# princeton-computational-imaging/Neural-Volume-Super-Resolution

Measured on AMD Instinct MI355X. Metric: rendered rays/sec (64+128 samples) at 800x800 Lego-like view, higher is better.
Workload: dtype f32 as 2 f16 limbs (3 MFMA products, f32 acc); 1 GPU; Blender-'lego'-like 800x800 view, 64 coarse + 128 fine samples, tri-plane decoder (3x800^2x48 + 32^2x48 planes, 4+4x128 MLP), 1 view per GPU per step; partition=view

## Files before the change

include/nvsr.h:

```cpp
#ifndef NVSR_H
#define NVSR_H
#include <stdint.h>

#ifdef __cplusplus
extern "C" {
#endif

typedef void* nvsr_stream_t;

typedef enum {
    NVSR_OK = 0,
    NVSR_ERR_SHAPE = 1,
    NVSR_ERR_LAUNCH = 2,
    NVSR_ERR_NULL = 3,
    NVSR_ERR_ALIGN = 4
} nvsr_status;

#define NVSR_PLANE_CHANNELS 48
#define NVSR_DEC_CHANNELS 128
#define NVSR_DEC_LAYERS 4
#define NVSR_DECODER_NATURAL_FLOATS 130564
#define NVSR_DECODER_PACKED_F32_FLOATS 130576
#define NVSR_DECODER_PACKED_FLOATS 453136
#define NVSR_DECODER_PACKED_BWD_FLOATS 487424
// ... 10 lines not shown

#define NVSR_ARITH_INHERIT (-1)
#define NVSR_ARITH_INVALID (-2)
#define NVSR_ARITH_F32 0
#define NVSR_ARITH_F16 1
#define NVSR_ARITH_F16X2 2
#define NVSR_ARITH_BF16X3 3
#define NVSR_ARITH_DEFAULT NVSR_ARITH_F16X2
int nvsr_get_decoder_arithmetic(void);
int nvsr_set_decoder_arithmetic(int mode);
int nvsr_set_range_flag(uint32_t* device_word);
uint32_t* nvsr_get_range_flag(void);
int nvsr_release_render_scratch(void);
int64_t nvsr_render_scratch_bytes(void);
int nvsr_internal_group_order(const int* trips, int64_t G, int S, int* out, nvsr_stream_t stream);
int nvsr_internal_copy_group_order(int* dst, int64_t G, nvsr_stream_t stream);
int nvsr_internal_live_order(int* live_n, int64_t N, int S, nvsr_stream_t stream);
int nvsr_internal_colour_order_bins(void);
int nvsr_internal_copy_live_counts(int* dst, int64_t N, nvsr_stream_t stream);
int nvsr_internal_point_order(const int* entries, const float* lists, const float* rays, int64_t N, int S, int bands, int* points, int* steps, int* offsets,
                              nvsr_stream_t stream);
int nvsr_internal_point_bands(void);
int nvsr_internal_copy_point_steps(int* dst, int64_t G, nvsr_stream_t stream);
int64_t nvsr_occupancy_words(int G);
int64_t nvsr_occupancy_workspace_floats(int G, int K);
int nvsr_occupancy_build(const nvsr_scene* scene, const float* packed_decoder, int G, int K, float threshold, int dilate, int arithmetic, uint32_t* grid,
                         float* workspace, nvsr_stream_t stream);
int nvsr_render_pass_occupancy_arith(const nvsr_scene* scene, const float* packed_decoder, int64_t N, int S, const float* rays, const float* z, int lindisp,
                                     int white_bkgd, float* rgb, float* disp, float* acc, float* weights, float* depth, const uint32_t* grid, int G, int arithmetic,
                                     nvsr_stream_t stream);
int nvsr_render_rays_occupancy_arith(const nvsr_scene* scene, const float* packed_coarse, const float* packed_fine, int64_t N, int Nc, int Nf,
                                     const float* rays, int lindisp, int white_bkgd, const float* t_rand, const float* u, float* rgb_c, float* disp_c,
                                     float* acc_c, float* rgb_f, float* disp_f, float* acc_f, float* workspace, const uint32_t* grid_coarse, int G_coarse,
                                     const uint32_t* grid_fine, int G_fine, int arithmetic, nvsr_stream_t stream);
int nvsr_internal_occupancy_probes(const nvsr_scene* scene, int G, int K, float* x, nvsr_stream_t stream);
int nvsr_internal_occupancy_cull(const nvsr_scene* scene, int64_t N, int S, const float* rays, const float* z, int lindisp, const uint32_t* grid, int G, int* kept,
                                 int* kept_n, nvsr_stream_t stream);
int nvsr_internal_copy_kept_counts(int* dst, int64_t N, nvsr_stream_t stream);
int nvsr_limb_gemm_probe(int arithmetic, int K, const float* W, const float* X, float* Y, nvsr_stream_t stream);
#define NVSR_CONV_ARITH_DEFAULT NVSR_ARITH_F16X2
int nvsr_get_conv_arithmetic(void);
int nvsr_set_conv_arithmetic(int mode);

int nvsr_plane_to_channel_last(const float* nchw, float* nhwc, int C, int H, int W, nvsr_stream_t stream);
int nvsr_plane_from_channel_last(const float* nhwc, float* nchw, int C, int H, int W, nvsr_stream_t stream);

// ... 349 lines not shown
```

neural-volume-super-resolution_amd/build.py:

```python
import glob
import os
import shutil
import subprocess

PKG_DIR = os.path.dirname(os.path.abspath(__file__))
CSRC = os.path.join(PKG_DIR, "csrc")
LIB_PATH = os.path.join(PKG_DIR, "libnvsr_hip.so")
HIPCC_FLAGS = ["--offload-arch=gfx950", "-O3", "-std=c++17", "-fPIC", "-shared", "-ffp-contract=off"]


def sources():
    return sorted(glob.glob(os.path.join(CSRC, "*.hip")))


STAMP_PATH = LIB_PATH + ".flags"


def _flag_stamp():
    extra = os.environ.get("NVSR_EXTRA_HIPCC_FLAGS", "").split()
    return " ".join(HIPCC_FLAGS) + " | " + " ".join("%s:%s" % kv for kv in sorted((k, ",".join(v)) for k, v in PER_FILE_FLAGS.items())) + " | " + " ".join(extra)


def _stamp_matches():
    try:
        with open(STAMP_PATH) as f:
            return f.read() == _flag_stamp()
    except OSError:
        return False


def _stale():
    if not os.path.exists(LIB_PATH) or not _stamp_matches():
        return True
    t = os.path.getmtime(LIB_PATH)
    deps = sources() + glob.glob(os.path.join(CSRC, "*.h")) + glob.glob(os.path.join(PKG_DIR, "..", "include", "*.h")) + [os.path.abspath(__file__)]
    return any(os.path.getmtime(p) > t for p in deps)


_PAIR_FLAGS = ["-fno-slp-vectorize", "-mllvm", "-pragma-unroll-threshold=1000000"]
_SR_FLAGS = ["-mllvm", "-enable-post-misched=0"]
PER_FILE_FLAGS = {"render3.hip": _PAIR_FLAGS, "decode_pair.hip": _PAIR_FLAGS, "decode_limb.hip": ["-fno-slp-vectorize"], "render_bwd_limb.hip": ["-fno-slp-vectorize"],
                  "sr.hip": _SR_FLAGS, "sr_bwd.hip": _SR_FLAGS}
OBJ_DIR = os.path.join(CSRC, "_obj")


def _compile_one(hipcc, src, verbose):
    obj = os.path.join(OBJ_DIR, os.path.basename(src) + ".o")
    deps = [src] + glob.glob(os.path.join(CSRC, "*.h")) + glob.glob(os.path.join(PKG_DIR, "..", "include", "*.h")) + [os.path.abspath(__file__)]
    stamp = obj + ".flags"
    same_flags = os.path.exists(stamp) and open(stamp).read() == _flag_stamp()
    if same_flags and os.path.exists(obj) and all(os.path.getmtime(d) <= os.path.getmtime(obj) for d in deps):
        return obj
    flags = [f for f in HIPCC_FLAGS if f != "-shared"] + PER_FILE_FLAGS.get(os.path.basename(src), [])
    flags += os.environ.get("NVSR_EXTRA_HIPCC_FLAGS", "").split()
    cmd = [hipcc] + flags + ["-c", src, "-o", obj]
    if verbose:
        print(" ".join(cmd))
    subprocess.check_call(cmd)
    with open(obj + ".flags", "w") as f:
        f.write(_flag_stamp())
    return obj


def build_extension(force=False, verbose=False, out_path=None):
# ... 54 lines not shown
```

neural-volume-super-resolution_amd/capi.py:

```python
import ctypes as C
import os

import torch

from .build import LIB_PATH as _DEFAULT_LIB_PATH

LIB_PATH = os.environ.get("NVSR_HIP_LIB", _DEFAULT_LIB_PATH)

PLANE_CHANNELS = 48
DEC_CHANNELS = 128
DECODER_NATURAL_FLOATS = 130564
DECODER_PACKED_FLOATS = 453136
DECODER_PACKED_BWD_FLOATS = 487424
MIP_NERF_NATURAL_FLOATS = 81092
MIP_NERF_RECORD_FLOATS = 767
MIP_NERF_GRAD_RECORD_FLOATS = 708
PE_NERF_NATURAL_FLOATS = 81476
PE_NERF_RECORD_FLOATS = 770
PE_NERF_GRAD_RECORD_FLOATS = 708
MSE_PAIR_MAX_ELEMS = 1 << 22

_STATUS = {1: "NVSR_ERR_SHAPE (argument out of the supported range)", 2: "NVSR_ERR_LAUNCH (kernel launch failed)",
           3: "NVSR_ERR_NULL (required pointer is NULL)", 4: "NVSR_ERR_ALIGN (pointer not 16-byte aligned)"}

# ... 158 lines not shown
    "nvsr_ray_points": ([_i64, _i, _vp, _vp, _vp, _vp], _i),
    "nvsr_render_shared_workspace_floats": ([_i64, _i, _i], _i64),
    "nvsr_render_rays_shared_arith": ([C.POINTER(Scene), _vp, _i64, _i, _i, _vp, _i, _i, _vp, _vp, _vp, _vp, _vp, _vp, _vp, _vp, _vp, _vp, _vp, _i, _vp], _i),
    "nvsr_shared_merge": ([_i64, _i, _i, _vp, _i, _vp, _vp, _vp, _vp, _vp, _vp], _i),
    "nvsr_release_render_scratch": ([], _i),
    "nvsr_render_scratch_bytes": ([], _i64),
    "nvsr_internal_group_order": ([_vp, _i64, _i, _vp, _vp], _i),
    "nvsr_internal_copy_group_order": ([_vp, _i64, _vp], _i),
    "nvsr_internal_live_order": ([_vp, _i64, _i, _vp], _i),
    "nvsr_internal_colour_order_bins": ([], _i),
    "nvsr_internal_copy_live_counts": ([_vp, _i64, _vp], _i),
    "nvsr_internal_point_bands": ([], _i),
    "nvsr_internal_copy_point_steps": ([_vp, _i64, _vp], _i),
    "nvsr_internal_point_order": ([_vp, _vp, _vp, _i64, _i, _i, _vp, _vp, _vp, _vp], _i),
    "nvsr_occupancy_words": ([_i], _i64),
    "nvsr_occupancy_workspace_floats": ([_i, _i], _i64),
    "nvsr_occupancy_build": ([C.POINTER(Scene), _vp, _i, _i, C.c_float, _i, _i, _vp, _vp, _vp], _i),
    "nvsr_render_pass_occupancy_arith": ([C.POINTER(Scene), _vp, _i64, _i, _vp, _vp, _i, _i, _vp, _vp, _vp, _vp, _vp, _vp, _i, _i, _vp], _i),
    "nvsr_render_rays_occupancy_arith": ([C.POINTER(Scene), _vp, _vp, _i64, _i, _i, _vp, _i, _i, _vp, _vp, _vp, _vp, _vp, _vp, _vp, _vp, _vp, _vp, _i, _vp, _i,
                                          _i, _vp], _i),
    "nvsr_internal_occupancy_probes": ([C.POINTER(Scene), _i, _i, _vp, _vp], _i),
    "nvsr_internal_occupancy_cull": ([C.POINTER(Scene), _i64, _i, _vp, _vp, _i, _vp, _i, _vp, _vp, _vp], _i),
    "nvsr_internal_copy_kept_counts": ([_vp, _i64, _vp], _i),
    "nvsr_set_sr_plane_interp": ([_i], _i),
    "nvsr_get_sr_plane_interp": ([], _i),
    "nvsr_set_sr_align_corners": ([_i], _i),
    "nvsr_get_sr_align_corners": ([], _i),
    "nvsr_render_pass_arith": ([C.POINTER(Scene), _vp, _i64, _i, _vp, _vp, _vp, _i, _vp, _vp, _vp, _vp, _vp, _vp, _i, _vp], _i),
    "nvsr_decode_rays_arith": ([C.POINTER(Scene), _vp, _i64, _i, _vp, _vp, _vp, _vp, _vp, _i, _vp], _i),
    "nvsr_render_rays_arith": ([C.POINTER(Scene), _vp, _vp, _i64, _i, _i, _vp, _i, _i, _vp, _vp, _vp, _vp, _vp, _vp, _vp, _vp, _vp,
                                _vp, _vp, _i, _vp], _i),
    "nvsr_render_pass_backward_gates_arith": ([C.POINTER(Scene), _vp, _vp, _i64, _i, _vp, _vp, _vp, _vp, C.POINTER(C.c_void_p), _vp, _vp, _i, _vp], _i),
    "nvsr_decoder_weight_grad_arith": ([_i64, _i, _vp, _vp, _i, _vp], _i),
    "nvsr_conv3x3_arith": ([_vp, _i, _i, _i, _vp, _i, _i, _vp, _vp, _i, _i, _vp], _i),
    "nvsr_conv3x3_dgrad_arith": ([_vp, _i, _i, _i, _vp, _i, _vp, _i, _i, _vp], _i),
    "nvsr_conv3x3_wgrad_arith": ([_vp, _vp, _i, _i, _i, _i, C.c_float, _vp, _vp, _i, _vp], _i),
    "nvsr_edsr_forward_batch_arith": ([_vp, _i, _i, _i, _i, _vp, _i, _i, _i, _i, _vp, _vp, _i, _vp], _i),
    "nvsr_edsr_forward_train_arith": ([_vp, _i, _i, _i, _vp, _i, _i, _i, _i, _vp, _vp, _i, _vp], _i),
    "nvsr_edsr_backward_arith": ([_vp, _i, _i, _i, _vp, _vp, _i, _i, _i, _i, _vp, _vp, _vp, _vp, _i, _vp], _i),
    "nvsr_planes_sr_arith": ([_vp, _i, _i, _i, _vp, _i, _i, _i, _i, _i, _fp, _vp, _vp, _vp, _vp, _i, _vp], _i),
    "nvsr_planes_sr_batch_arith": ([C.POINTER(C.c_void_p), _i, _i, _i, _i, _vp, _i, _i, _i, _i, _i, _fp, _vp, _vp, C.POINTER(C.c_void_p), _vp, _i, _vp], _i),
    "nvsr_planes_sr_train_arith": ([_vp, _i, _i, _i, _vp, _i, _i, _i, _i, _i, _fp, _vp, _vp, _vp, _vp, _vp, _i, _vp], _i),
    "nvsr_planes_sr_backward_arith": ([_i, _i, _i, _vp, _vp, _i, _i, _i, _i, _i, _fp, _vp, _vp, _vp, _vp, _vp, _i, _vp], _i),
    "nvsr_planes_sr_batch_ex": ([C.POINTER(C.c_void_p), _i, _i, _i, _i, _vp, _i, _i, _i, _i, _i, _fp, _vp, _vp, C.POINTER(C.c_void_p), _vp, _i, _i, _i, _vp], _i),
    "nvsr_planes_sr_batch_keep_floats": ([_i, _i, _i, _i, _i, _i, _i, _i, _fp], _i64),
    "nvsr_planes_sr_batch_workspace_floats": ([_i, _i, _i, _i, _i, _i, _i, _i, _fp], _i64),
# ... 248 lines not shown
```

neural-volume-super-resolution_amd/csrc/colour_order.h:

```cpp
#pragma once
#include "tile_pair.h"

namespace nvsr {

constexpr int ORDER_SHIFT = 12, ORDER_RAYS = 1 << ORDER_SHIFT, ORDER_BINS = 32;
constexpr int ORDER_MAX_S = 1 << (31 - ORDER_SHIFT);
static_assert(ORDER_RAYS % RAYS2 == 0, "a block of the ray order is a whole number of workgroups");

#ifndef NVSR_POINT_BANDS
#define NVSR_POINT_BANDS 0
#endif
constexpr int POINT_BANDS = NVSR_POINT_BANDS, POINT_NONE = -1, POINT_VIEW_FLOATS = 2 * HALF_C;
static_assert(RAYS2 <= 256 && ORDER_MAX_S <= (1 << 24), "a slot and a list index share an entry");

struct LiveLists { float* z; float* w; int* n; int* slot; int* trip; int* pts; int* steps; float* views; };

struct KeptLists { int* idx; int* n; int* slot; int* trip; };

enum class PassRoute { Fused, TwoPhase, Occupancy };
PassRoute acquire_pass_scratch(int64_t N, int S, hipStream_t stream, bool raw_out, bool want_kept, bool launch, LiveLists& live, KeptLists& kept);
void launch_colour_order(const LiveLists& ll, int64_t N, int S, hipStream_t stream);
void launch_kept_order(const KeptLists& kl, int64_t N, int S, hipStream_t stream);
void launch_point_order(const LiveLists& ll, const float* rays_nf, int64_t N, int S, hipStream_t stream);

}
```

neural-volume-super-resolution_amd/csrc/colour_order.hip:

```cpp
#include "colour_order.h"
#include "occupancy.h"
#include "nvsr_internal.h"

#include <cstdlib>
#include <mutex>
#include <vector>

namespace nvsr {

constexpr int SORT_TPB = 1024, SORT_WAVES = SORT_TPB / 64, SORT_ROUNDS = 4, SORT_MAX = SORT_TPB * SORT_ROUNDS;
template <int NKEYS>
__device__ __forceinline__ void counting_sort(const int (&key)[SORT_ROUNDS], int nkeys, int n, int (&start)[SORT_ROUNDS], int (&place)[SORT_ROUNDS],
                                              int (&len)[SORT_ROUNDS]) {
    static_assert(NKEYS <= SORT_TPB, "one thread per key sums the tables");
    __shared__ int cnt_s[NKEYS * SORT_WAVES];
    __shared__ int tot_s[NKEYS], start_s[NKEYS];
    const int wave = threadIdx.x >> 6, lane = threadIdx.x & 63;
    const unsigned long long below = (1ull << lane) - 1ull;
    for (int b = 0; b <= nkeys; ++b) {
        int c = 0;
#pragma unroll
        for (int r = 0; r < SORT_ROUNDS; ++r) c += __popcll(__ballot(key[r] == b));
        if (lane == 0) cnt_s[b * SORT_WAVES + wave] = c;
    }
// ... 145 lines not shown
    if (base + j < nsteps * RAYS2) out[base + j] = POINT_NONE;
    if (j == 0) { steps[blockIdx.x] = nsteps; offs[blockIdx.x] = (int)blockIdx.x * S; }
    __syncthreads();
    for (int t = 0; t < nsteps; ++t) {
        const int e = out[t * RAYS2 + j];
        const bool valid = e != POINT_NONE;
        const int sl = (int)((unsigned)e >> 24), kk = e & 0xffffff;
        kmin_s[j] = 0x7fffffff; cnt_s[j] = 0;
        __syncthreads();
        if (valid) { atomicMin(&kmin_s[sl], kk); atomicAdd(&cnt_s[sl], 1); }
        __syncthreads();
        int total;
        start_s[j] = scan(cnt_s[j], 0, total);
        __syncthreads();
        stage_s[valid ? start_s[sl] + (kk - kmin_s[sl]) : j] = e;
        __syncthreads();
        out[t * RAYS2 + j] = stage_s[j];
    }
}

namespace {
enum { LISTS, GROUP, POINTS, VIEWS, KEPT, KEPT_GROUP, N_BUFFERS };
struct Buffer { void* p; size_t bytes; };
struct Launch { int64_t N; int* n; int* steps; int64_t kept_N; int* kept; };
struct Scratch { int device; hipStream_t stream; Buffer buf[N_BUFFERS]; Launch last; };
std::mutex g_live_mutex;
std::vector<Scratch> g_live;

Scratch* find_scratch(int device, hipStream_t stream) {
    for (Scratch& c : g_live)
        if (c.device == device && c.stream == stream) return &c;
    return nullptr;
}

bool grow(Scratch& e, int which, size_t bytes) {
    Buffer& b = e.buf[which];
    if (b.bytes >= bytes) return true;
    if (b.p) (void)hipFree(b.p);
    b = Buffer{};
    e.last = Launch{};
    void* p = nullptr;
    if (hipMalloc(&p, bytes) != hipSuccess) { (void)hipGetLastError(); return false; }
    b = Buffer{p, bytes};
    return true;
}

int64_t groups_of(int64_t N) { return (N + RAYS2 - 1) / RAYS2; }
// ... 55 lines not shown
    live.w = live.z + rows;
    live.n = reinterpret_cast<int*>(live.w + rows);
    live.slot = static_cast<int*>(e->buf[GROUP].p);
    live.trip = live.slot + G;
    const size_t npts = G * RAYS2 * (size_t)S;
    if (!env_starts("NVSR_COLOUR_POINTS", '0') && G * (size_t)S <= 0x7fffffffu && grow(*e, POINTS, (npts + 2 * G) * sizeof(int)) &&
        grow(*e, VIEWS, G * RAYS2 * POINT_VIEW_FLOATS * sizeof(float))) {
        live.pts = static_cast<int*>(e->buf[POINTS].p);
        live.steps = live.pts + npts;
        live.views = static_cast<float*>(e->buf[VIEWS].p);
    }
    PassRoute route = PassRoute::TwoPhase;
    if (want_kept && grow(*e, KEPT_GROUP, 2 * G * sizeof(int)) && grow(*e, KEPT, (rows + (size_t)N) * sizeof(int))) {
        kept.idx = static_cast<int*>(e->buf[KEPT].p);
        kept.n = kept.idx + rows;
        kept.slot = static_cast<int*>(e->buf[KEPT_GROUP].p);
        kept.trip = kept.slot + G;
        route = PassRoute::Occupancy;
    }
    if (launch) e->last = route == PassRoute::Occupancy ? Launch{N, live.n, live.steps, N, kept.n} : Launch{N, live.n, live.steps, e->last.kept_N, e->last.kept};
    return route;
}

static void launch_orders(int* n, int* trip, int* slot, int64_t N, int S, hipStream_t stream) {
    launch_live_order(n, N, S, env_starts("NVSR_COLOUR_ORDER", '0') ? 0 : ORDER_BINS, trip, stream);
    launch_group_order(trip, groups_of(N), S, slot, stream);
}
void launch_kept_order(const KeptLists& kl, int64_t N, int S, hipStream_t stream) { launch_orders(kl.n, kl.trip, kl.slot, N, S, stream); }
void launch_colour_order(const LiveLists& ll, int64_t N, int S, hipStream_t stream) { launch_orders(ll.n, ll.trip, ll.slot, N, S, stream); }

void launch_point_order(const LiveLists& ll, const float* rays_nf, int64_t N, int S, hipStream_t stream) {
    launch_point_order(ll.n, ll.z, rays_nf, N, S, POINT_BANDS, ll.pts, ll.steps, ll.steps + groups_of(N), stream);
}

}

using namespace nvsr;

extern "C" int nvsr_internal_colour_order_bins(void) { return ORDER_BINS; }
extern "C" int nvsr_internal_live_order(int* live_n, int64_t N, int S, nvsr_stream_t stream) {
    if (!live_n) return NVSR_ERR_NULL;
    if (N < 1 || S < 1 || S >= ORDER_MAX_S || (N + ORDER_RAYS - 1) / ORDER_RAYS > 0x7fffffff) return NVSR_ERR_SHAPE;
    launch_live_order(live_n, N, S, ORDER_BINS, nullptr, (hipStream_t)stream);
    return NVSR_CHECK_LAUNCH();
}
extern "C" int nvsr_internal_copy_live_counts(int* dst, int64_t N, nvsr_stream_t stream) {
    return copy_left_behind(dst, N, stream, [N](const Scratch& c) { return c.last.N == N ? c.last.n : nullptr; });
}
extern "C" int nvsr_internal_group_order(const int* trips, int64_t G, int S, int* out, nvsr_stream_t stream) {
    if (!trips || !out) return NVSR_ERR_NULL;
    if (G < 1 || G > 0x7fffffff || S < 1 || S >= ORDER_MAX_S) return NVSR_ERR_SHAPE;
    launch_group_order(trips, G, S, out, (hipStream_t)stream);
    return NVSR_CHECK_LAUNCH();
}
extern "C" int nvsr_internal_copy_group_order(int* dst, int64_t G, nvsr_stream_t stream) {
    return copy_left_behind(dst, 2 * G, stream, [G](const Scratch& c) { return c.last.n && groups_of(c.last.N) == G ? static_cast<int*>(c.buf[GROUP].p) : nullptr; });
}

extern "C" int nvsr_internal_point_bands(void) { return POINT_BANDS; }
extern "C" int nvsr_internal_point_order(const int* entries, const float* lists, const float* rays, int64_t N, int S, int bands, int* points, int* steps, int* offsets,
                                         nvsr_stream_t stream) {
    if (!entries || !lists || !points || !steps || !offsets) return NVSR_ERR_NULL;
    const int64_t G = (N + RAYS2 - 1) / RAYS2;
    if (N < 1 || S < 1 || S >= ORDER_MAX_S || G * S > 0x7fffffff) return NVSR_ERR_SHAPE;
    launch_point_order(entries, lists, rays, N, S, bands, points, steps, offsets, (hipStream_t)stream);
    return NVSR_CHECK_LAUNCH();
}
extern "C" int nvsr_internal_copy_point_steps(int* dst, int64_t G, nvsr_stream_t stream) {
    return copy_left_behind(dst, G, stream, [G](const Scratch& c) { return c.last.n && groups_of(c.last.N) == G ? c.last.steps : nullptr; });
}
// ... 31 lines not shown
```

neural-volume-super-resolution_amd/csrc/decode_limb.hip:

```cpp
#include <type_traits>

#include "limb_core.h"
#include "nvsr_internal.h"

#ifndef L3_REC_LATE
#define L3_REC_LATE 0
#endif
#ifndef L3_ABLATE
#define L3_ABLATE 0
#endif

namespace nvsr {

constexpr int L3_TPB = 256, L3_WAVES = L3_TPB / 64, L3_PTS = L3_WAVES * 32;
template <int LF>
struct L3 {
    static constexpr int SLOT = 3 * kb_words(LF);
    static constexpr int SMALL = 2 * SLOT;
    static constexpr int LDS = SMALL + SMALL_FLOATS;
};
static_assert(2 * L3<3>::LDS * 4 <= 160 * 1024, "two workgroups per CU");
#ifdef NVSR_RECORD_SAMPLE_MAJOR
template <int LF> constexpr bool L3_STAGED = false;
#else
// ... 10 lines not shown
};

template <int NKB, int LF = 3>
__device__ __forceinline__ const unsigned* ringl_issue(RingL& rs, int kb0) {
    unsigned* dst = rs.lds + rs.slot * L3<LF>::SLOT;
    constexpr int PIECES = NKB * 4 * LF;
    static_assert(PIECES % L3_WAVES == 0, "chunk must split evenly over the waves");
#pragma unroll
    for (int i = 0; i < PIECES / L3_WAVES; ++i)
        __builtin_amdgcn_raw_ptr_buffer_load_lds(rs.rsrc, (__attribute__((address_space(3))) void*)(dst + (i * L3_WAVES + rs.wave) * 256), 16,
                                                 (int)rs.voff, kb0 * kb_words(LF) * 4 + i * (L3_WAVES * 1024), 0, 0);
    rs.slot ^= 1;
    return dst;
}
template <int YOUNGER = 0>
__device__ __forceinline__ void ringl_sync() {
#if !(L3_ABLATE & 4)
    if constexpr (YOUNGER == 0) asm volatile("s_waitcnt vmcnt(0)" ::: "memory");
    else asm volatile("s_waitcnt vmcnt(%0)" : : "n"(YOUNGER) : "memory");
#endif
    __syncthreads();
}

template <int LF>
__device__ __forceinline__ void bias_relu(const f32x16 (&acc)[4], const float* bias, int h, f32x16 (&act)[4], float nsc) {
#pragma unroll
    for (int g = 0; g < 16; ++g) {
        const f32x4 b = *reinterpret_cast<const f32x4*>(bias + g * 8 + h * 4);
#pragma unroll
        for (int j = 0; j < 4; ++j) {
            if constexpr (LF == 2) {
                float v;
                asm("v_fma_f32 %0, -%1, %2, %3\n\tv_max_i32 %0, 0, %0" : "=v"(v) : "v"(acc[g >> 2][4 * (g & 3) + j]), "s"(nsc), "v"(b[j]));
                act[g >> 2][4 * (g & 3) + j] = v;
            } else act[g >> 2][4 * (g & 3) + j] = fmaxf(acc[g >> 2][4 * (g & 3) + j] + b[j], 0.0f);
        }
    }
}
__device__ __forceinline__ void publish_gates(const f32x16 (&act)[4], unsigned* __restrict__ rec, int layer) {
    unsigned m0 = 0u, m1 = 0u;
#pragma unroll
    for (int ib = 0; ib < 4; ++ib)
#pragma unroll
        for (int r = 0; r < 16; r += 4) {
            unsigned t0, t1, t2, t3;
            unsigned& m = ib < 2 ? m0 : m1;
            asm("v_med3_i32 %1, %5, 0, 1\n\tv_med3_i32 %2, %6, 0, 1\n\tv_med3_i32 %3, %7, 0, 1\n\tv_med3_i32 %4, %8, 0, 1\n\t"
                "v_lshl_or_b32 %0, %1, %9, %0\n\tv_lshl_or_b32 %0, %2, %10, %0\n\tv_lshl_or_b32 %0, %3, %11, %0\n\tv_lshl_or_b32 %0, %4, %12, %0"
                : "+v"(m), "=&v"(t0), "=&v"(t1), "=&v"(t2), "=&v"(t3)
                : "v"(act[ib][r]), "v"(act[ib][r + 1]), "v"(act[ib][r + 2]), "v"(act[ib][r + 3]), "n"(gate_bit(ib, r)), "n"(gate_bit(ib, r + 1)),
                  "n"(gate_bit(ib, r + 2)), "n"(gate_bit(ib, r + 3)));
        }
    typedef unsigned u32x2 __attribute__((ext_vector_type(2)));
    *reinterpret_cast<u32x2*>(rec + 2 * layer) = u32x2{m0, m1};
}

template <bool MASKS, bool RECORD, int LF>
__device__ __forceinline__ void decode_step_limb(const SceneDev& sc, RingL& rs, const float* small, float px, float py, float pz, const Taps& vt_,
                                                 float (&raw)[4], unsigned* __restrict__ gates, const DecRecord& rec, long q, bool rec_ok, float nsc,
                                                 float* stage = nullptr, long q0 = 0, int nvalid = 0) {
    auto scaled = [](Taps t) {
// ... 247 lines not shown
```

neural-volume-super-resolution_amd/csrc/limb_core.h:

```cpp
#pragma once
#include "decode_core.h"

namespace nvsr {

typedef unsigned u32x4 __attribute__((ext_vector_type(4)));
typedef __bf16 bf16x8 __attribute__((ext_vector_type(8)));
typedef __bf16 bf16x2_t __attribute__((ext_vector_type(2)));
typedef float f32x2_t __attribute__((ext_vector_type(2)));
typedef _Float16 f16x8 __attribute__((ext_vector_type(8)));
typedef _Float16 f16x2_t __attribute__((ext_vector_type(2)));

#define NVSR_CX __host__ __device__ __attribute__((always_inline)) constexpr
#define NVSR_INL __attribute__((always_inline))
NVSR_CX int limb_products(int limbs) { return limbs == 3 ? 6 : limbs == 1 ? 1 : 3; }
NVSR_CX int limb_w(int limbs, int p) { return limbs == 3 ? (p < 3 ? 0 : p < 5 ? 1 : 2) : limbs == 1 ? 0 : (p < 2 ? 0 : 1); }
NVSR_CX int limb_x(int limbs, int p) { return limbs == 3 ? (p == 0 ? 2 : p == 1 ? 1 : p == 2 ? 0 : p == 3 ? 1 : 0) : limbs == 1 ? 0 : (p == 0 ? 1 : 0); }

constexpr int KB_RGB0 = 0;
constexpr int KB_RGB1 = 12;
constexpr int KB_DEN0 = 36;
constexpr int KB_DEN1 = 39;
constexpr int KB_TOTAL = 63;
constexpr int kb_words(int limbs) { return 4 * limbs * 256; }
constexpr int P_LIMB3 = NVSR_DECODER_PACKED_F32_FLOATS;
// ... 149 lines not shown
                __builtin_amdgcn_sched_barrier(0);
#if defined(R3_ABLATE) && (R3_ABLATE & 128)
                if (p < LIMBS) { fn.v[p] = fa.v[p]; fn.v[p][0] ^= (unsigned)(q + 1); }
#else
                if (p < LIMBS) { const int t_ = LIMBS - 1 - p; fn.v[t_] = wv[(((q + 1) % NQ) * LIMBS + t_) * 64]; }
#endif
                if (kb + 1 < NKB) {
                    split_slice<LIMBS>(ob * NP + p, [&](int i) { return src(kb + 1, i); }, nxt, sp);
                    if constexpr (HAS_GATE) { if ((ob * NP + p) % NP == 0 && (ob * NP + p) / NP < 4) gate(kb + 1, (ob * NP + p) / NP, nxt.v[0][(ob * NP + p) / NP]); }
                } else if constexpr (HAS_TAIL) tail(ob * NP + p, nxt);
                side(q * NP + p);
                __builtin_amdgcn_sched_barrier(0);
            }
#pragma unroll
            for (int t = 0; t < LIMBS; ++t) fa.v[t] = fn.v[t];
        }
        if (kb + 1 < NKB || HAS_TAIL) {
#pragma unroll
            for (int t = 0; t < LIMBS; ++t) cur.v[t] = nxt.v[t];
        }
    }
}

}
```

neural-volume-super-resolution_amd/csrc/nvsr_internal.h:

```cpp
#pragma once
#include "nvsr_common.h"

extern "C" {
int nvsr_render_pass2_launch(const nvsr_scene* scene, const float* packed_decoder, int64_t N, int S, const float* rays, const float* z, const float* noise, int white_bkgd,
                             float* rgb, float* disp, float* acc, float* weights, float* depth, float* raw_out, nvsr_stream_t stream);
int nvsr_render_pass3_launch(int limbs, const nvsr_scene* scene, const float* packed_decoder, int64_t N, int S, const float* rays, const float* z, const float* noise,
                             int white_bkgd, float* rgb, float* disp, float* acc, float* weights, float* depth, float* raw_out, nvsr_stream_t stream);
int nvsr_render_pass3_coarse_z_launch(int limbs, const nvsr_scene* scene, const float* packed_decoder, int64_t N, int S, const float* rays, int lindisp, const float* noise,
                                      int white_bkgd, float* rgb, float* disp, float* acc, float* weights, float* depth, float* raw_out, nvsr_stream_t stream);
int nvsr_pack_decoder_limbs_launch(const float* natural, float* packed, nvsr_stream_t stream);
int nvsr_pack_decoder_bwd_limbs_launch(const float* natural, float* packed_bwd, nvsr_stream_t stream);
int nvsr_decode_rays_limb_launch(int limbs, const nvsr_scene* scene, const float* packed_decoder, int64_t N, int S, const float* rays, const float* z, float* raw,
                                 uint32_t* gates, float* record, nvsr_stream_t stream);
int nvsr_decode_rays_pair_launch(const nvsr_scene* scene, const float* packed_decoder, int64_t N, int S, const float* rays, const float* z, float* raw, uint32_t* gates,
                                 nvsr_stream_t stream);
int nvsr_render_pass_backward_gates_limb_launch(int limbs, const nvsr_scene* scene, const float* packed_decoder, const float* packed_bwd, int64_t N, int S, const float* rays,
                                                const float* z, const float* g_raw, const uint32_t* gates, float* const* grad_planes, float* view_ws, float* record,
                                                nvsr_stream_t stream);
int nvsr_render_pass_backward_rows_limb_launch(int limbs, const nvsr_scene* scene, const float* packed_decoder, const float* packed_bwd, int64_t N, int S, const float* rays,
                                               const float* z, const float* g_raw, const uint32_t* gates, float* const* rows, float* view_ws, float* record,
                                               nvsr_stream_t stream);
int nvsr_internal_resolve_decoder_arith(int arithmetic);
int nvsr_internal_resolve_render_arith(int arithmetic);
int nvsr_internal_parse_arith_env(const char* name, int dflt, int conv);
void nvsr_internal_reserve_render_scratch(int64_t N, int S, nvsr_stream_t stream);
int nvsr_internal_conv_route(int Cin, int Cout, int H, int W, int arithmetic, int rows_per_tile, int* family, int* region, unsigned* packed_kinds);
}

namespace nvsr {

inline int check_scene(const nvsr_scene* s) {
    if (!s) return NVSR_ERR_NULL;
    for (int d = 0; d < 4; ++d) {
        if (!s->planes[d]) return NVSR_ERR_NULL;
        if (!aligned16(s->planes[d])) return NVSR_ERR_ALIGN;
        if (s->ph[d] < 1 || s->pw[d] < 1 || (int64_t)s->ph[d] * s->pw[d] * NVSR_PLANE_CHANNELS >= (int64_t)1 << 31) return NVSR_ERR_SHAPE;
    }
    return NVSR_OK;
}

}
```

neural-volume-super-resolution_amd/csrc/render3.hip:

```cpp
#include "pair_core.h"

#include "colour_order.h"
#include "occupancy.h"
#include "nvsr_internal.h"

namespace nvsr {

template <int LZ>
__device__ __forceinline__ void render_pass3_body(const SceneDev& sc, const float* __restrict__ packed, long N, int S,
                                                  const float* __restrict__ rays, const float* __restrict__ z, int lindisp,
                                                  const float* __restrict__ noise, int white,
                                                  float* __restrict__ rgb, float* __restrict__ disp,
                                                  float* __restrict__ acc, float* __restrict__ weights,
                                                  float* __restrict__ depth, float* __restrict__ raw_out, unsigned* __restrict__ flag,
                                                  float* __restrict__ live_z = nullptr, float* __restrict__ live_w = nullptr,
                                                  int* __restrict__ live_n = nullptr, const int* __restrict__ group_slot = nullptr,
                                                  const int* __restrict__ pts = nullptr, const int* __restrict__ pt_steps = nullptr, float* views = nullptr,
                                                  const int* __restrict__ kept = nullptr, const int* __restrict__ kept_n = nullptr) {
    constexpr int LIMBS = LZ & 7;
    constexpr bool ZCOMP = (LZ & 8) != 0;
    constexpr int PHASE = (LZ >> 4) & 7;
    constexpr bool FUSED = PHASE == 0, KEPT = PHASE == 4, DENSITY = PHASE == 1 || KEPT, POINTS = PHASE == 3, COLOUR = PHASE == 2 || POINTS;
    constexpr bool F16 = limb_f16(LIMBS);
    using L = Lds3<LIMBS>;
// ... 893 lines not shown
using namespace nvsr;

extern "C" int nvsr_limb_gemm_probe(int arithmetic, int K, const float* W, const float* X, float* Y, nvsr_stream_t stream) {
    if (!W || !X || !Y) return NVSR_ERR_NULL;
    if (K < 16 || K % 16) return NVSR_ERR_SHAPE;
    if (arithmetic == NVSR_ARITH_F32) hipLaunchKernelGGL(limb_gemm_probe_kernel<0>, dim3(1), dim3(64), 0, (hipStream_t)stream, K, W, X, Y);
    else if (arithmetic == NVSR_ARITH_BF16X3) hipLaunchKernelGGL(limb_gemm_probe_kernel<3>, dim3(1), dim3(64), 0, (hipStream_t)stream, K, W, X, Y);
    else if (arithmetic == NVSR_ARITH_F16X2) hipLaunchKernelGGL(limb_gemm_probe_kernel<2>, dim3(1), dim3(64), 0, (hipStream_t)stream, K, W, X, Y);
    else return NVSR_ERR_SHAPE;
    return NVSR_CHECK_LAUNCH();
}

extern "C" int nvsr_pack_decoder_limbs_launch(const float* natural, float* packed, nvsr_stream_t stream) {
    unsigned* out = reinterpret_cast<unsigned*>(packed);
    const int n3 = KB_TOTAL * kb_words(3), n2 = KB_TOTAL * kb_words(2);
    hipLaunchKernelGGL(pack_decoder_limbs_kernel<3>, dim3((n3 + 255) / 256), dim3(256), 0, (hipStream_t)stream, natural, out + P_LIMB3);
    hipLaunchKernelGGL(pack_decoder_limbs_kernel<2>, dim3((n2 + 255) / 256), dim3(256), 0, (hipStream_t)stream, natural, out + P_LIMB2);
    return NVSR_CHECK_LAUNCH();
}

struct PassArgs { const nvsr_scene* scene; const float* packed; int64_t N; int S; const float *rays, *z; int lindisp; const float* noise; int white;
                  float *rgb, *disp, *acc, *weights, *depth, *raw_out; hipStream_t stream; };
struct OccLaunch { const uint32_t* grid; int G; KeptLists kept; };
template <int LIMBS>
static int launch_pass3(const PassArgs& a, const LiveLists* ll, const OccLaunch* occ) {
    const SceneDev sc = to_dev(a.scene);
    unsigned* flag = nvsr_get_range_flag();
    auto launch = [&](auto kernel, auto... args) {
        hipLaunchKernelGGL(kernel, dim3((unsigned)((a.N + RAYS2 - 1) / RAYS2)), dim3(TPB2), 0, a.stream, sc, a.packed, (long)a.N, a.S, a.rays, args...);
    };
    if (ll) {
        if (occ) {
            if constexpr (LIMBS == 1) return NVSR_ERR_SHAPE;
            else {
                const KeptLists& kl = occ->kept;
                launch_occupancy_cull(sc, a.N, a.S, a.rays, a.z, a.lindisp, occ->grid, occ->G, kl.idx, kl.n, a.stream);
                launch_kept_order(kl, a.N, a.S, a.stream);
                if (a.weights && hipMemsetAsync(a.weights, 0, (size_t)a.N * (size_t)a.S * sizeof(float), a.stream) != hipSuccess) return NVSR_ERR_LAUNCH;
                if (a.z) launch(render_pass3_density_kept_kernel<LIMBS>, a.z, a.disp, a.acc, a.weights, a.depth, flag, ll->z, ll->w, ll->n, kl.slot, kl.idx, kl.n);
                else launch(render_pass3_density_kept_z_kernel<LIMBS>, a.lindisp, a.disp, a.acc, a.weights, a.depth, flag, ll->z, ll->w, ll->n, kl.slot, kl.idx, kl.n);
            }
        } else if (a.z) launch(render_pass3_density_kernel<LIMBS>, a.z, a.noise, a.disp, a.acc, a.weights, a.depth, flag, ll->z, ll->w, ll->n);
        else launch(render_pass3_density_z_kernel<LIMBS>, a.lindisp, a.noise, a.disp, a.acc, a.weights, a.depth, flag, ll->z, ll->w, ll->n);
        launch_colour_order(*ll, a.N, a.S, a.stream);
        if (ll->pts) {
            launch_point_order(*ll, a.z ? a.rays : nullptr, a.N, a.S, a.stream);
            if (a.z) launch(render_pass3_points_kernel<LIMBS>, a.white, a.rgb, a.acc, flag, ll->z, ll->w, ll->n, ll->slot, ll->pts, ll->steps, ll->views);
            else launch(render_pass3_points_z_kernel<LIMBS>, a.lindisp, a.white, a.rgb, a.acc, flag, ll->z, ll->w, ll->n, ll->slot, ll->pts, ll->steps, ll->views);
        } else if (a.z) launch(render_pass3_colour_kernel<LIMBS>, a.white, a.rgb, a.acc, flag, ll->z, ll->w, ll->n, ll->slot);
        else launch(render_pass3_colour_z_kernel<LIMBS>, a.lindisp, a.white, a.rgb, a.acc, flag, ll->z, ll->w, ll->n, ll->slot);
    } else if (!a.z) launch(render_pass3_coarse_z_kernel<LIMBS>, a.lindisp, a.noise, a.white, a.rgb, a.disp, a.acc, a.weights, a.depth, a.raw_out, flag);
    else if (a.weights) launch(render_pass3_coarse_kernel<LIMBS>, a.z, a.noise, a.white, a.rgb, a.disp, a.acc, a.weights, a.depth, a.raw_out, flag);
    else launch(render_pass3_kernel<LIMBS>, a.z, a.noise, a.white, a.rgb, a.disp, a.acc, a.depth, a.raw_out, flag);
    return NVSR_CHECK_LAUNCH();
}
static int launch_pass3(int limbs, const PassArgs& a, const uint32_t* grid = nullptr, int G = 0) {
    LiveLists lists; OccLaunch occ{grid, G, {}};
    const PassRoute route = acquire_pass_scratch(a.N, a.S, a.stream, a.raw_out != nullptr, grid != nullptr, true, lists, occ.kept);
    const LiveLists* ll = route == PassRoute::Fused ? nullptr : &lists;
    const OccLaunch* oc = route == PassRoute::Occupancy ? &occ : nullptr;
    return limbs == 3 ? launch_pass3<3>(a, ll, oc) : limbs == 1 ? launch_pass3<1>(a, ll, oc) : launch_pass3<2>(a, ll, oc);
}

extern "C" int nvsr_render_pass3_launch(int limbs, const nvsr_scene* scene, const float* packed_decoder, int64_t N, int S, const float* rays, const float* z,
// ... 32 lines not shown
```

Baseline: 7.801 million rays/s.

## Add single-tile density kernel with LDS-resident early layers and staggered gathers

Adds a dedicated density-pass kernel for the two-limb path. It keeps the first density layers' weights resident in LDS and double-buffers the later K-blocks through a two-slot ring using buffer-to-LDS DMA. Half the waves prefetch the next sample's tri-plane gather ahead of the matrix work, to overlap memory latency with MFMA work. It is on by default for the two-phase route with an env switch back to the old kernel. It also records which density kernel ran. The cost is a large LDS footprint at one block per CU and more per-step barriers.

```diff
diff --git a/include/nvsr.h b/include/nvsr.h
--- a/include/nvsr.h
+++ b/include/nvsr.h
@@ -56,6 +56,7 @@
                               nvsr_stream_t stream);
 int nvsr_internal_point_bands(void);
 int nvsr_internal_copy_point_steps(int* dst, int64_t G, nvsr_stream_t stream);
+int nvsr_internal_density_kernel(nvsr_stream_t stream);
 int64_t nvsr_occupancy_words(int G);
 int64_t nvsr_occupancy_workspace_floats(int G, int K);
 int nvsr_occupancy_build(const nvsr_scene* scene, const float* packed_decoder, int G, int K, float threshold, int dilate, int arithmetic, uint32_t* grid,
diff --git a/neural-volume-super-resolution_amd/build.py b/neural-volume-super-resolution_amd/build.py
--- a/neural-volume-super-resolution_amd/build.py
+++ b/neural-volume-super-resolution_amd/build.py
@@ -39,7 +39,7 @@
 
 _PAIR_FLAGS = ["-fno-slp-vectorize", "-mllvm", "-pragma-unroll-threshold=1000000"]
 _SR_FLAGS = ["-mllvm", "-enable-post-misched=0"]
-PER_FILE_FLAGS = {"render3.hip": _PAIR_FLAGS, "decode_pair.hip": _PAIR_FLAGS, "decode_limb.hip": ["-fno-slp-vectorize"], "render_bwd_limb.hip": ["-fno-slp-vectorize"],
+PER_FILE_FLAGS = {"render3.hip": _PAIR_FLAGS, "decode_pair.hip": _PAIR_FLAGS, "decode_limb.hip": ["-fno-slp-vectorize"], "density_tile.hip": ["-fno-slp-vectorize"], "render_bwd_limb.hip": ["-fno-slp-vectorize"],
                   "sr.hip": _SR_FLAGS, "sr_bwd.hip": _SR_FLAGS}
 OBJ_DIR = os.path.join(CSRC, "_obj")
 
diff --git a/neural-volume-super-resolution_amd/capi.py b/neural-volume-super-resolution_amd/capi.py
--- a/neural-volume-super-resolution_amd/capi.py
+++ b/neural-volume-super-resolution_amd/capi.py
@@ -204,6 +204,7 @@
     "nvsr_internal_occupancy_probes": ([C.POINTER(Scene), _i, _i, _vp, _vp], _i),
     "nvsr_internal_occupancy_cull": ([C.POINTER(Scene), _i64, _i, _vp, _vp, _i, _vp, _i, _vp, _vp, _vp], _i),
     "nvsr_internal_copy_kept_counts": ([_vp, _i64, _vp], _i),
+    "nvsr_internal_density_kernel": ([_vp], _i),
     "nvsr_set_sr_plane_interp": ([_i], _i),
     "nvsr_get_sr_plane_interp": ([], _i),
     "nvsr_set_sr_align_corners": ([_i], _i),
diff --git a/neural-volume-super-resolution_amd/csrc/colour_order.h b/neural-volume-super-resolution_amd/csrc/colour_order.h
--- a/neural-volume-super-resolution_amd/csrc/colour_order.h
+++ b/neural-volume-super-resolution_amd/csrc/colour_order.h
@@ -19,6 +19,7 @@
 
 enum class PassRoute { Fused, TwoPhase, Occupancy };
 PassRoute acquire_pass_scratch(int64_t N, int S, hipStream_t stream, bool raw_out, bool want_kept, bool launch, LiveLists& live, KeptLists& kept);
+void note_density_kernel(hipStream_t stream, int which);
 void launch_colour_order(const LiveLists& ll, int64_t N, int S, hipStream_t stream);
 void launch_kept_order(const KeptLists& kl, int64_t N, int S, hipStream_t stream);
 void launch_point_order(const LiveLists& ll, const float* rays_nf, int64_t N, int S, hipStream_t stream);
diff --git a/neural-volume-super-resolution_amd/csrc/colour_order.hip b/neural-volume-super-resolution_amd/csrc/colour_order.hip
--- a/neural-volume-super-resolution_amd/csrc/colour_order.hip
+++ b/neural-volume-super-resolution_amd/csrc/colour_order.hip
@@ -191,7 +191,7 @@
 namespace {
 enum { LISTS, GROUP, POINTS, VIEWS, KEPT, KEPT_GROUP, N_BUFFERS };
 struct Buffer { void* p; size_t bytes; };
-struct Launch { int64_t N; int* n; int* steps; int64_t kept_N; int* kept; };
+struct Launch { int64_t N; int* n; int* steps; int64_t kept_N; int* kept; int density; };
 struct Scratch { int device; hipStream_t stream; Buffer buf[N_BUFFERS]; Launch last; };
 std::mutex g_live_mutex;
 std::vector<Scratch> g_live;
@@ -293,6 +293,13 @@
     return route;
 }
 
+void note_density_kernel(hipStream_t stream, int which) {
+    int device = 0;
+    if (hipGetDevice(&device) != hipSuccess) return;
+    std::lock_guard<std::mutex> lock(g_live_mutex);
+    if (Scratch* e = find_scratch(device, stream)) e->last.density = which;
+}
+
 static void launch_orders(int* n, int* trip, int* slot, int64_t N, int S, hipStream_t stream) {
     launch_live_order(n, N, S, env_starts("NVSR_COLOUR_ORDER", '0') ? 0 : ORDER_BINS, trip, stream);
     launch_group_order(trip, groups_of(N), S, slot, stream);
@@ -317,6 +324,13 @@
 }
 extern "C" int nvsr_internal_copy_live_counts(int* dst, int64_t N, nvsr_stream_t stream) {
     return copy_left_behind(dst, N, stream, [N](const Scratch& c) { return c.last.N == N ? c.last.n : nullptr; });
+}
+extern "C" int nvsr_internal_density_kernel(nvsr_stream_t stream) {
+    int device = 0;
+    if (hipGetDevice(&device) != hipSuccess) return -1;
+    std::lock_guard<std::mutex> lock(g_live_mutex);
+    const Scratch* c = find_scratch(device, (hipStream_t)stream);
+    return c && c->last.n ? c->last.density : -1;
 }
 extern "C" int nvsr_internal_group_order(const int* trips, int64_t G, int S, int* out, nvsr_stream_t stream) {
     if (!trips || !out) return NVSR_ERR_NULL;
diff --git a/neural-volume-super-resolution_amd/csrc/decode_limb.hip b/neural-volume-super-resolution_amd/csrc/decode_limb.hip
--- a/neural-volume-super-resolution_amd/csrc/decode_limb.hip
+++ b/neural-volume-super-resolution_amd/csrc/decode_limb.hip
@@ -56,21 +56,6 @@
     __syncthreads();
 }
 
-template <int LF>
-__device__ __forceinline__ void bias_relu(const f32x16 (&acc)[4], const float* bias, int h, f32x16 (&act)[4], float nsc) {
-#pragma unroll
-    for (int g = 0; g < 16; ++g) {
-        const f32x4 b = *reinterpret_cast<const f32x4*>(bias + g * 8 + h * 4);
-#pragma unroll
-        for (int j = 0; j < 4; ++j) {
-            if constexpr (LF == 2) {
-                float v;
-                asm("v_fma_f32 %0, -%1, %2, %3\n\tv_max_i32 %0, 0, %0" : "=v"(v) : "v"(acc[g >> 2][4 * (g & 3) + j]), "s"(nsc), "v"(b[j]));
-                act[g >> 2][4 * (g & 3) + j] = v;
-            } else act[g >> 2][4 * (g & 3) + j] = fmaxf(acc[g >> 2][4 * (g & 3) + j] + b[j], 0.0f);
-        }
-    }
-}
 __device__ __forceinline__ void publish_gates(const f32x16 (&act)[4], unsigned* __restrict__ rec, int layer) {
     unsigned m0 = 0u, m1 = 0u;
 #pragma unroll
diff --git a/neural-volume-super-resolution_amd/csrc/density_tile.hip b/neural-volume-super-resolution_amd/csrc/density_tile.hip
--- /dev/null
+++ b/neural-volume-super-resolution_amd/csrc/density_tile.hip
@@ -0,0 +1,238 @@
+#include "pair_core.h"
+
+#include "nvsr_internal.h"
+
+#ifndef DT_ABLATE
+#define DT_ABLATE 0
+#endif
+#ifndef DT_STAGGER
+#define DT_STAGGER 1
+#endif
+
+namespace nvsr {
+
+constexpr int DT_TPB = 512, DT_WAVES = DT_TPB / 64, DT_RAYS = DT_WAVES * 32;
+static_assert(DT_RAYS == RAYS2, "the grid is the tile-pair kernels'");
+struct LdsTile {
+    static constexpr int SLOT = 4 * kb_words(2);
+    static constexpr int RES = 2 * SLOT;
+    static constexpr int RES_KB = KB_DEN1 + 8 - KB_DEN0;
+    static constexpr int SMALL = RES + RES_KB * kb_words(2);
+    static constexpr int TOTAL = SMALL + SMALL_FLOATS;
+};
+static_assert(KB_DEN1 - KB_DEN0 == 3 && LdsTile::RES_KB == 11, "density layer 0 is one block of three K-blocks, layer 1 two of four");
+static_assert(LdsTile::TOTAL * 4 <= 160 * 1024, "LDS budget");
+
+template <int NKB>
+__device__ __forceinline__ void tile_copy(const Ring3<2>& rs, unsigned* dst, int kb0) {
+    constexpr int PIECES = NKB * 4 * 2;
+    static_assert(PIECES % DT_WAVES == 0, "a copy must split evenly over the waves");
+#pragma unroll
+    for (int i = 0; i < PIECES / DT_WAVES; ++i)
+        __builtin_amdgcn_raw_ptr_buffer_load_lds(rs.rsrc, (__attribute__((address_space(3))) void*)(dst + (i * DT_WAVES + rs.wave) * 256), 16,
+                                                 (int)rs.voff, kb0 * kb_words(2) * 4 + i * (DT_WAVES * 1024), 0, R3_DMA_AUX);
+}
+template <int NKB>
+__device__ __forceinline__ const unsigned* tile_issue(Ring3<2>& rs, int kb0) {
+    static_assert(NKB * kb_words(2) <= LdsTile::SLOT, "a chunk fits the slot");
+    unsigned* dst = rs.lds + rs.slot * LdsTile::SLOT;
+#if !(DT_ABLATE & 1)
+    tile_copy<NKB>(rs, dst, kb0);
+#endif
+    rs.slot ^= 1;
+    return dst;
+}
+__device__ __forceinline__ void tile_sync() {
+#if !(DT_ABLATE & 4)
+    asm volatile("s_waitcnt vmcnt(0)" ::: "memory");
+    __syncthreads();
+#endif
+}
+
+struct TileD { float T, dep, ac, zc, zn; float raw[4]; };
+
+template <int ZCOMP>
+__device__ __forceinline__ void density_tile_body(const SceneDev& sc, const float* __restrict__ packed, long N, int S, const float* __restrict__ rays,
+                                                  const float* __restrict__ z, int lindisp, const float* __restrict__ noise, float* __restrict__ disp,
+                                                  float* __restrict__ acc_out, float* __restrict__ weights, float* __restrict__ depth,
+                                                  unsigned* __restrict__ flag, float* __restrict__ live_z, float* __restrict__ live_w,
+                                                  int* __restrict__ live_n) {
+    using L = LdsTile;
+    __shared__ __attribute__((aligned(16))) unsigned lds[L::TOTAL];
+    NVSR_RACE_PROBE_DELAY(lds);
+    Ring3<2> rs{__builtin_amdgcn_make_buffer_rsrc(const_cast<float*>(packed + limb_region(2)), 0, KB_TOTAL * kb_words(2) * 4, 0x00020000),
+                lds, 0, __builtin_amdgcn_readfirstlane((int)(threadIdx.x >> 6)), (int)(threadIdx.x & 63), ring3_voff<2>(threadIdx.x)};
+    float* ldsf = reinterpret_cast<float*>(lds);
+    for (int i = threadIdx.x; i < SMALL_FLOATS; i += DT_TPB) {
+        float v = packed[P_SMALL + i] * (i < S_ALPHA_W ? F16_X_SCALE : i < S_HEAD_B ? F16_HEAD_SCALE : 1.0f);
+        if (i >= S_HEAD_B && i < S_HEAD_B + 4) v += packed[P_SMALL + S_F16_POISON];
+        ldsf[L::SMALL + i] = v;
+    }
+    const float* small = ldsf + L::SMALL;
+    float nsc = -F16_ACC_UNSCALE;
+    asm volatile("" : "+s"(nsc));
+    tile_copy<L::RES_KB>(rs, lds + L::RES, KB_DEN0);
+
+    const unsigned nblk = gridDim.x, xcd = blockIdx.x & 7u, per = nblk >> 3, rem = nblk & 7u;
+    const unsigned blk = xcd * per + (xcd < rem ? xcd : rem) + (blockIdx.x >> 3);
+    long ray = (long)blk * DT_RAYS + rs.wave * 32 + (rs.lane & 31);
+    const bool valid = ray < N;
+    if (!valid) ray = N - 1;
+    const float* r = rays + ray * 11;
+    const float ox = r[0], oy = r[1], oz = r[2], dx = r[3], dy = r[4], dz = r[5], near = r[6], far = r[7];
+    const float nrm = sqrtf(__fadd_rn(__fadd_rn(__fmul_rn(dx, dx), __fmul_rn(dy, dy)), __fmul_rn(dz, dz)));
+    const float* zrow = ZCOMP ? nullptr : z + ray * S;
+    auto depth_of = [&](int k) NVSR_INL -> float {
+        if constexpr (ZCOMP) return coarse_depth(near, far, k, S, lindisp);
+        else return zrow[k];
+    };
+    TileD t;
+    t.T = 1.0f; t.dep = t.ac = 0.0f;
+    t.zc = depth_of(0);
+    int cursor = 0;
+    const bool ahead = DT_STAGGER && rs.wave >= DT_WAVES / 2;
+
+    tile_sync();
+    const unsigned* cw = tile_issue<4>(rs, KB_DEN1 + 8);
+
+    f32x16 acc[4], act[4];
+    float D[HALF_C], F[HALF_C];
+    Limbs<2> cur, fa;
+    SplitPend tp;
+    auto feat = [](const float (&f)[HALF_C]) { return [&f](int kb, int i) { return f[8 * kb + i]; }; };
+    auto hid = [](const f32x16 (&a)[4], int kb0) { return [&a, kb0](int kb, int i) { const int k = kb0 + kb; return a[k >> 1][8 * (k & 1) + i]; }; };
+    auto none = [](int) {};
+    auto tail_of = [&tp](const f32x16 (&a)[4], int kb) {
+        return [&a, kb, &tp](int slice, Limbs<2>& nxt) { split_slice<2>(slice, [&a, kb](int i) { return a[kb >> 1][8 * (kb & 1) + i]; }, nxt, tp); };
+    };
+#define DT_FENCE                                                                                    \
+    asm volatile("" : "+v"(acc[0]), "+v"(acc[1]), "+v"(acc[2]), "+v"(acc[3]) : : "memory");         \
+    __builtin_amdgcn_sched_barrier(0);
+#define DT_RES_BLOCK(KB_OFF, NKB, ZERO, FIRST, SRC, TAIL)                                          \
+    {                                                                                              \
+        if (FIRST) { auto s_ = SRC; split_all<2>([&](int i) { return s_(0, i); }, cur); }          \
+        limb_block<2, NKB, ZERO, true>(lds + L::RES + (KB_OFF) * kb_words(2), lane, acc, cur, fa, SRC, none, TAIL);      \
+        DT_FENCE                                                                                   \
+    }
+#define DT_BLOCK(ZERO, FIRST, SRC, KB_NEXT, TAIL)                                                  \
+    {                                                                                              \
+        tile_sync();                                                                               \
+        const unsigned* nw = tile_issue<4>(rs, KB_NEXT);                                           \
+        if (FIRST) { auto s_ = SRC; split_all<2>([&](int i) { return s_(0, i); }, cur); }          \
+        limb_block<2, 4, ZERO, true>(cw, lane, acc, cur, fa, SRC, none, TAIL);                     \
+        cw = nw;                                                                                   \
+        DT_FENCE                                                                                   \
+    }
+#if DT_ABLATE & 8
+#define DT_RELU(VEC) { _Pragma("unroll") for (int ib = 0; ib < 4; ++ib) act[ib] = acc[ib]; }
+#else
+#define DT_RELU(VEC) bias_relu<2>(acc, small + S_BIAS + (VEC) * HID, h, act, nsc);
+#endif
+
+    for (int s = 0; s < S; ++s) {
+        asm volatile("" : "+v"(rs.voff), "+v"(rs.lane));
+        const int lane = rs.lane, h = lane >> 5;
+        const bool last = (s + 1 == S);
+        t.zn = depth_of(last ? s : s + 1);
+        const float nz = noise ? noise[ray * S + s] : 0.0f;
+        auto gather_d = [&](float zc) NVSR_INL {
+            const float n0 = norm_coord(__fadd_rn(ox, __fmul_rn(dx, zc)), sc.lo[0], sc.range[0]);
+            const float n1 = norm_coord(__fadd_rn(oy, __fmul_rn(dy, zc)), sc.lo[1], sc.range[1]);
+            const float n2 = norm_coord(__fadd_rn(oz, __fmul_rn(dz, zc)), sc.lo[2], sc.range[2]);
+#pragma unroll
+            for (int p = 0; p < 3; ++p) {
+                Taps tap = pos_taps2(sc, p, n0, n1, n2);
+                tap.nw *= F16_X_SCALE; tap.ne *= F16_X_SCALE; tap.sw *= F16_X_SCALE; tap.se *= F16_X_SCALE;
+#if DT_ABLATE & 2
+                for (int c = 0; c < HALF_C; ++c) F[c] = tap.nw * (float)(c + h);
+#else
+                gather24(sc.plane[p], tap, h, F);
+#endif
+#pragma unroll
+                for (int c = 0; c < HALF_C; ++c) {
+                    D[c] = p == 0 ? F[c] : p == 1 ? __fadd_rn(D[c], F[c]) : div3(__fadd_rn(D[c], F[c]));
+                    asm volatile("" : "+v"(D[c]));
+                }
+                __builtin_amdgcn_sched_barrier(0);
+            }
+        };
+        if (!ahead || s == 0) gather_d(t.zc);
+        DT_RES_BLOCK(0, 3, true, true, feat(D), NoTail{})
+        DT_RELU(0)
+        DT_RES_BLOCK(3, 4, true, true, hid(act, 0), tail_of(act, 4))
+        DT_RES_BLOCK(7, 4, false, false, hid(act, 4), NoTail{})
+        DT_RELU(1)
+        if (ahead) gather_d(t.zn);
+        DT_BLOCK(true, true, hid(act, 0), KB_DEN1 + 12, tail_of(act, 4))
+        DT_BLOCK(false, false, hid(act, 4), KB_DEN1 + 16, NoTail{})
+        DT_RELU(2)
+        DT_BLOCK(true, true, hid(act, 0), KB_DEN1 + 20, tail_of(act, 4))
+        DT_BLOCK(false, false, hid(act, 4), KB_DEN1 + 8, NoTail{})
+        DT_RELU(3)
+        {
+            float hd[1];
+            head_dots<1>(small + S_ALPHA_W, h, act, hd);
+            t.raw[3] = hd[0] + small[S_HEAD_B];
+        }
+        composite_weight(t, nrm, nz, last);
+        const float w = t.raw[3];
+        const bool live = !(w == 0.0f);
+        if (lane < 32 && valid) {
+            if (weights) weights[ray * S + s] = w;
+            if (live) { live_z[ray * S + cursor] = ZCOMP ? __int_as_float(s) : t.zc; live_w[ray * S + cursor] = w; }
+        }
+        cursor += live;
+        t.zc = t.zn;
+    }
+#undef DT_RELU
+#undef DT_BLOCK
+#undef DT_RES_BLOCK
+#undef DT_FENCE
+    asm volatile("s_waitcnt vmcnt(0)" ::: "memory");
+
+    if (rs.lane < 32 && valid) {
+        const float q = t.dep / t.ac;
+        disp[ray] = 1.0f / ((q != q) ? q : fmaxf(1e-10f, q));
+        acc_out[ray] = t.ac;
+        if (depth) depth[ray] = t.dep;
+        live_n[ray] = cursor;
+        if (flag && !(fabsf(t.ac) <= 3.0e38f)) __hip_atomic_fetch_or(flag, 1u, __ATOMIC_RELAXED, __HIP_MEMORY_SCOPE_AGENT);
+    }
+}
+
+__global__ __launch_bounds__(DT_TPB, 1) void density_tile_kernel(SceneDev sc, const float* __restrict__ packed, long N, int S, const float* __restrict__ rays,
+                                                                 const float* __restrict__ z, const float* __restrict__ noise, float* __restrict__ disp,
+                                                                 float* __restrict__ acc, float* __restrict__ weights, float* __restrict__ depth,
+                                                                 unsigned* __restrict__ flag, float* __restrict__ live_z, float* __restrict__ live_w,
+                                                                 int* __restrict__ live_n) {
+#if defined(__HIP_DEVICE_COMPILE__)
+    density_tile_body<0>(sc, packed, N, S, rays, z, 0, noise, disp, acc, weights, depth, flag, live_z, live_w, live_n);
+#endif
+}
+__global__ __launch_bounds__(DT_TPB, 1) void density_tile_z_kernel(SceneDev sc, const float* __restrict__ packed, long N, int S, const float* __restrict__ rays,
+                                                                   int lindisp, const float* __restrict__ noise, float* __restrict__ disp,
+                                                                   float* __restrict__ acc, float* __restrict__ weights, float* __restrict__ depth,
+                                                                   unsigned* __restrict__ flag, float* __restrict__ live_z, float* __restrict__ live_w,
+                                                                   int* __restrict__ live_n) {
+#if defined(__HIP_DEVICE_COMPILE__)
+    density_tile_body<1>(sc, packed, N, S, rays, nullptr, lindisp, noise, disp, acc, weights, depth, flag, live_z, live_w, live_n);
+#endif
+}
+
+}
+
+using namespace nvsr;
+
+extern "C" int nvsr_density_tile_launch(const nvsr_scene* scene, const float* packed_decoder, int64_t N, int S, const float* rays, const float* z, int lindisp,
+                                        const float* noise, float* disp, float* acc, float* weights, float* depth, float* live_z, float* live_w, int* live_n,
+                                        nvsr_stream_t stream) {
+    const int64_t blocks = (N + DT_RAYS - 1) / DT_RAYS;
+    if (N < 1 || blocks > 0x7fffffff) return NVSR_ERR_SHAPE;
+    const SceneDev sc = to_dev(scene);
+    unsigned* flag = nvsr_get_range_flag();
+    if (z) hipLaunchKernelGGL(density_tile_kernel, dim3((unsigned)blocks), dim3(DT_TPB), 0, (hipStream_t)stream, sc, packed_decoder, (long)N, S, rays, z, noise,
+                              disp, acc, weights, depth, flag, live_z, live_w, live_n);
+    else hipLaunchKernelGGL(density_tile_z_kernel, dim3((unsigned)blocks), dim3(DT_TPB), 0, (hipStream_t)stream, sc, packed_decoder, (long)N, S, rays, lindisp,
+                            noise, disp, acc, weights, depth, flag, live_z, live_w, live_n);
+    return NVSR_CHECK_LAUNCH();
+}
diff --git a/neural-volume-super-resolution_amd/csrc/limb_core.h b/neural-volume-super-resolution_amd/csrc/limb_core.h
--- a/neural-volume-super-resolution_amd/csrc/limb_core.h
+++ b/neural-volume-super-resolution_amd/csrc/limb_core.h
@@ -195,4 +195,20 @@
     }
 }
 
-}
+template <int LF>
+__device__ __forceinline__ void bias_relu(const f32x16 (&acc)[4], const float* bias, int h, f32x16 (&act)[4], float nsc) {
+#pragma unroll
+    for (int g = 0; g < 16; ++g) {
+        const f32x4 b = *reinterpret_cast<const f32x4*>(bias + g * 8 + h * 4);
+#pragma unroll
+        for (int j = 0; j < 4; ++j) {
+            if constexpr (LF == 2) {
+                float v;
+                asm("v_fma_f32 %0, -%1, %2, %3\n\tv_max_i32 %0, 0, %0" : "=v"(v) : "v"(acc[g >> 2][4 * (g & 3) + j]), "s"(nsc), "v"(b[j]));
+                act[g >> 2][4 * (g & 3) + j] = v;
+            } else act[g >> 2][4 * (g & 3) + j] = fmaxf(acc[g >> 2][4 * (g & 3) + j] + b[j], 0.0f);
+        }
+    }
+}
+
+}
diff --git a/neural-volume-super-resolution_amd/csrc/nvsr_internal.h b/neural-volume-super-resolution_amd/csrc/nvsr_internal.h
--- a/neural-volume-super-resolution_amd/csrc/nvsr_internal.h
+++ b/neural-volume-super-resolution_amd/csrc/nvsr_internal.h
@@ -20,6 +20,9 @@
 int nvsr_render_pass_backward_rows_limb_launch(int limbs, const nvsr_scene* scene, const float* packed_decoder, const float* packed_bwd, int64_t N, int S, const float* rays,
                                                const float* z, const float* g_raw, const uint32_t* gates, float* const* rows, float* view_ws, float* record,
                                                nvsr_stream_t stream);
+int nvsr_density_tile_launch(const nvsr_scene* scene, const float* packed_decoder, int64_t N, int S, const float* rays, const float* z, int lindisp,
+                             const float* noise, float* disp, float* acc, float* weights, float* depth, float* live_z, float* live_w, int* live_n,
+                             nvsr_stream_t stream);
 int nvsr_internal_resolve_decoder_arith(int arithmetic);
 int nvsr_internal_resolve_render_arith(int arithmetic);
 int nvsr_internal_parse_arith_env(const char* name, int dflt, int conv);
diff --git a/neural-volume-super-resolution_amd/csrc/render3.hip b/neural-volume-super-resolution_amd/csrc/render3.hip
--- a/neural-volume-super-resolution_amd/csrc/render3.hip
+++ b/neural-volume-super-resolution_amd/csrc/render3.hip
@@ -939,6 +939,11 @@
 struct PassArgs { const nvsr_scene* scene; const float* packed; int64_t N; int S; const float *rays, *z; int lindisp; const float* noise; int white;
                   float *rgb, *disp, *acc, *weights, *depth, *raw_out; hipStream_t stream; };
 struct OccLaunch { const uint32_t* grid; int G; KeptLists kept; };
+constexpr bool DENSITY_ONE_TILE_DEFAULT = true;
+static bool density_one_tile() {
+    const char* e = getenv("NVSR_DENSITY_ONE_TILE");
+    return e && (e[0] == '0' || e[0] == '1') ? e[0] == '1' : DENSITY_ONE_TILE_DEFAULT;
+}
 template <int LIMBS>
 static int launch_pass3(const PassArgs& a, const LiveLists* ll, const OccLaunch* occ) {
     const SceneDev sc = to_dev(a.scene);
@@ -957,6 +962,10 @@
                 if (a.z) launch(render_pass3_density_kept_kernel<LIMBS>, a.z, a.disp, a.acc, a.weights, a.depth, flag, ll->z, ll->w, ll->n, kl.slot, kl.idx, kl.n);
                 else launch(render_pass3_density_kept_z_kernel<LIMBS>, a.lindisp, a.disp, a.acc, a.weights, a.depth, flag, ll->z, ll->w, ll->n, kl.slot, kl.idx, kl.n);
             }
+        } else if (LIMBS == 2 && density_one_tile()) {
+            if (int e = nvsr_density_tile_launch(a.scene, a.packed, a.N, a.S, a.rays, a.z, a.lindisp, a.noise, a.disp, a.acc, a.weights, a.depth, ll->z, ll->w, ll->n,
+                                                 (nvsr_stream_t)a.stream)) return e;
+            note_density_kernel(a.stream, 1);
         } else if (a.z) launch(render_pass3_density_kernel<LIMBS>, a.z, a.noise, a.disp, a.acc, a.weights, a.depth, flag, ll->z, ll->w, ll->n);
         else launch(render_pass3_density_z_kernel<LIMBS>, a.lindisp, a.noise, a.disp, a.acc, a.weights, a.depth, flag, ll->z, ll->w, ll->n);
         launch_colour_order(*ll, a.N, a.S, a.stream);
```

After: 7.946 million rays/s, median of 6. 1.02x the previous value.
